# OpenRendererBenchmark/libYafaRay

Hardware: AMD Instinct MI355X
Metric: Mrays/sec (primary+secondary) on the path-tracing hot path (higher is better)
Workload: dtype f32; 1 GPU; 1M-tri diffuse Cornell-box soup 512x512 64spp primary+1-bounce (BASELINE.json metric config); triangles=1000000, width=512, height=512, spp=64, bounces=1, lights=1, parallelism=pixel-tile shard x1, film_reduce=none, kd_nodes=2803313, kd_leaf_refs=3155999, kd_max_depth=27

## Files before the change

libyafaray_amd/csrc/yafgpu_wavefront.h:

```cpp
#pragma once

namespace yafgpu {

constexpr int kWfRecs = 32;

struct WfArgs
{
	RenderArgs ra;
	float4 *state; uint32_t cap;
	float4 *results;
	uint32_t n_paths, pixel_begin, n_pixels;
	const uint32_t *pix_prefix;
	int frames;
	int frame_recs, has_glossy;
	int pix_listed;
	uint32_t *pix_xy;
	const uint32_t *q_closest_in, *q_shadow_in, *q_resume_in;
	uint32_t *q_closest_out, *q_shadow_out, *q_resume_out;
	uint32_t *verdict;
	float4 *shadow_filt;
	int replay, replay_lights;
	int ev_m;
	float4 *hit_cache; int hit_k;
	uint32_t *ev_flags;
// ... 1221 lines not shown
				if(!second && (gl & kGlSecond))
				{
					FREC(P, 9) = f4(gcol, f9.w);
					FREC(P, 6) = f4(v3(f6), fbits((gl & ~kGlSecond) | kGlOnSecond));
					wf_start_level(a, slot, c, v3(f2), v3(FREC(P, 3)));
					return W_PARK_CLOSEST;
				}
				if(second)
				{
					const float m_alpha = FREC(P, 1).x;
					alpha_p = rp.bg_transp_refract ? m_alpha + (1.f - m_alpha) * alpha : 1.f;
				}
			}
			else gcol = c3(f9) + (integ * c3(f10)) * f10.w;
			const int ns = (int)(gl & 0xffu) + 1, gsam = (int)((gl >> 8) & 0xffu);
			c.level = P;
			if(ns < gsam)
			{
				FREC(P, 9) = f4(gcol, f9.w);
				FREC(P, 6) = f4(v3(f6), fbits((uint32_t)ns | ((uint32_t)gsam << 8)));
				if(alpha_p != f0.w) FREC(P, 0) = f4(c3(f0), alpha_p);
				return W_GLOSSY_NEXT;
			}
			c.col = c3(f0) + gcol * (1.f / (float)gsam);
			VSET(3, f4(v3(f2), f9.w)); VSET(4, f4(v3(f6), 0.f)); VSET(5, FREC(P, 7)); VSET(6, FREC(P, 8));
			if(YAFGPU_FEAT_TEXTURE && a.ra.sc.tex.nodes != nullptr) REC(22) = FREC(P, 11);
			if(YAFGPU_FEAT_TEXTURE && a.ra.sc.tex.has_bump) REC(24) = FREC(P, 12);
			REC(19) = make_float4(0.f, 0.f, a.ev_m > 1 ? REC(19).z : 0.f, alpha_p);
			return W_RECURSE_SPEC;
		}
		if(flags & ((flags & 2u) ? 8u : 4u))
		{
			const yafgpu_material &pm = a.ra.sc.mats[ubits(FREC(P, 4).w)];
			integ = integ * beer_transmittance(pm.beer_sigma, FREC(P, 3).w);
		}
		if(!(flags & 2u))
		{
			const Col col_p = c3(f0) + integ * c3(FREC(P, 4));
			if(flags & 1u)
			{
				FREC(P, 0) = f4(col_p, f0.w);
				FREC(P, 2) = f4(v3(f2), fbits(2u | (flags & 8u) | (flags & 0xf00u)));
				wf_start_level(a, slot, c, wf_transp_origin(a.ra.sc.mats[ubits(FREC(P, 4).w)], v3(f2), v3(FREC(P, 3)), P + 1), v3(FREC(P, 3)));
				return W_PARK_CLOSEST;
			}
			c.col = col_p; alpha = f0.w;
		}
		else
		{
			const float4 f1 = FREC(P, 1);
			c.col = c3(f0) + integ * c3(f1);
			alpha = rp.bg_transp_refract ? f1.w + (1.f - f1.w) * alpha : 1.f;
		}
		c.level = P;
	}
}
#undef FREC

YG_DEV int wf_advance(const WfArgs &a, uint32_t slot, uint32_t pixel_sample, uint32_t sampling_offs, uint32_t ordinal, const float4 ans, float result[4], int &out_mask)
{
	Ctl c = load_ctl(a, slot);
	const bool beside = YAFGPU_FEAT_LIGHTS && c.pc == kPcAfterBoth;
	int where = (YAFGPU_FEAT_LIGHTS && (c.pc == kPcAfterShadow || beside)) ? W_AFTER_SHADOW : W_AFTER_CLOSEST;
	Hot h; hot_init(h);
	uint32_t w_last = 0u;
	float alpha = 0.f;
	uint2 verdict = make_uint2(0u, 0u), verdict2 = verdict;
	if(where == W_AFTER_SHADOW)
	{
		const uint32_t w = a.verdict[slot >> 3], sh = (slot & 7u) << 2;
		verdict = make_uint2((w >> sh) & 1u, (w >> (sh + 1u)) & 1u);
		verdict2 = make_uint2((w >> (sh + 2u)) & 1u, (w >> (sh + 3u)) & 1u);
		hot_preload(a, slot, h, c.stage != kStPrimary);
		if(YAFGPU_FEAT_LIGHTS && !beside)
		{
			const uint32_t w14 = ubits(h.r14.w);
			const int li = (int)(w14 & 0xffu), l_end = (int)((w14 >> 8) & 0xffu), is = (int)(w14 >> 20);
			bool more = li + 1 < l_end;
			if(YAFGPU_FEAT_AO && !more && li < l_end && li >= a.ra.sc.n_lights) more = is + 1 < ao_n_samples(a.ra.rp, wf_div(a, slot, c.level).division);
			else if(!more && li < l_end)
			{
				const yafgpu_light &light = a.ra.sc.lights[li];
				more = !light_is_dirac(light.type) && is + 1 < dl_area_samples(a.ra, light, wf_div(a, slot, c.level).division);
			}
			if(more) { if(c.dl_on_sp0) VNEED(3); else VNEED(7); }
		}
	}
	int pend2 = (YAFGPU_FEAT_LIGHTS && YAFGPU_FEAT_MULTI) ? c.mask2 : 0;
	c.mask2 = 0;
	if(beside)
	{
		where = st_after_shadow(a, slot, h, verdict);
		if(where == W_DL_NEXT) where = st_dl_next(a, slot, h, c.level);
		if(YAFGPU_FEAT_MULTI && where == W_DL_EVAL && pend2)
		{
			where = st_after_shadow(a, slot, h, verdict2, true, pend2);
			pend2 = 0;
			if(where == W_DL_NEXT) where = st_dl_next(a, slot, h, c.level);
		}
		if(where == W_DL_DONE) where = st_dl_done(a, slot, h, c, true);
		if(where == W_NEXT_VERTEX) where = W_AFTER_CLOSEST;
	}
	if(where == W_AFTER_CLOSEST) where = st_after_closest(a, slot, h, c, ordinal, ans, beside);
	if(YAFGPU_FEAT_LIGHTS && !a.vtx_lds && where == W_DL_NEXT) { if(c.dl_on_sp0) VNEED(3); else VNEED(7); }
	if(YAFGPU_FEAT_LIGHTS)
	{
		if(where == W_AFTER_SHADOW) where = st_after_shadow(a, slot, h, verdict);
		bool second = false;
		uint32_t w2 = 0u;
		while(where == W_DL_NEXT || where == W_DL_EVAL)
		{
			if(where == W_DL_NEXT) where = st_dl_next(a, slot, h, c.level);
			else if(YAFGPU_FEAT_MULTI && pend2) { where = st_after_shadow(a, slot, h, verdict2, true, pend2); pend2 = 0; }
			else
			{
				int m = 0;
				const int r = st_dl_eval(a, slot, h, c, pixel_sample, sampling_offs, m, second, w2);
				if(!second)
				{
					where = r;
					if(r == W_PARK_SHADOW)
					{
						out_mask = m;
						w_last = ubits(HGET(14).w);
						if(YAFGPU_FEAT_MULTI && a.multi)
						{
							const int li = (int)(w_last & 0xffu), l_end = (int)((w_last >> 8) & 0xffu), is = (int)(w_last >> 20);
							int n;
							if(YAFGPU_FEAT_AO && li >= a.ra.sc.n_lights) n = ao_n_samples(a.ra.rp, wf_div(a, slot, c.level).division);
							else
							{
								const yafgpu_light &light = a.ra.sc.lights[li];
								n = light_is_dirac(light.type) ? 1 : dl_area_samples(a.ra, light, wf_div(a, slot, c.level).division);
							}
							const bool same = is + 1 < n;
							if(same || li + 1 < l_end) { second = true; w2 = pack_dlc(same ? li : li + 1, l_end, 0, same ? is + 1 : 0); where = W_DL_EVAL; }
						}
					}
				}
				else
				{
					if(r == W_PARK_SHADOW) { c.mask2 = m; out_mask |= m << 2; w_last = w2; }
					where = W_PARK_SHADOW;
				}
			}
		}
	}
	if(where == W_DL_DONE) where = st_dl_done(a, slot, h, c, false);
	if(YAFGPU_FEAT_LIGHTS && where == W_PARK_SHADOW) where = st_beside(a, slot, h, c, pixel_sample, sampling_offs, ordinal, w_last);
	if(where == W_EXTEND) where = st_extend(a, slot, h, c);
	if(where == W_START_PATH) where = st_start_path(a, slot, h, c, pixel_sample, sampling_offs, ordinal);
	if(where == W_RECURSE) where = st_recurse(a, slot, h, c);
#if YAFGPU_FEAT_RECURSE
	for(;;)
	{
		if(where == W_GLOSSY_NEXT) where = st_glossy_next(a, slot, c, pixel_sample, sampling_offs);
		if(where == W_RECURSE_SPEC) where = st_recurse_spec(a, slot, h, c);
		if(where != W_RETURN) break;
		where = st_return(a, slot, h, c, alpha);
		if(where != W_GLOSSY_NEXT && where != W_RECURSE_SPEC) break;
	}
#else
	if(where == W_RETURN) where = st_return(a, slot, h, c, alpha);
#endif
	if(where != W_FINISH) hot_flush(a, slot, h, where == W_PARK_CLOSEST);
#if YAFGPU_FEAT_LIGHTS
	if(where != W_FINISH)
	{
		const bool sampler_later = c.stage == kStPrimary || (c.stage == kStFirst ? 1 : c.depth + 1) < a.ra.rp.bounces;
		vtx_flush(a, slot, h, where == W_PARK_SHADOW && sampler_later);
	}
#endif
	if(where == W_PARK_CLOSEST) { c.pc = kPcAfterClosest; REC(13) = f4(c.col, fbits(pack_ctl(c))); return kReqClosest; }
	if(where == W_PARK_SHADOW) { c.pc = kPcAfterShadow; REC(13) = f4(c.col, fbits(pack_ctl(c))); return kReqShadow; }
	if(where == W_PARK_BOTH) { c.pc = kPcAfterBoth; REC(13) = f4(c.col, fbits(pack_ctl(c))); return kReqBoth; }
	if(a.ra.rp.bg_transp) alpha = smax(alpha, 0.f);
	result[0] = c.col.r; result[1] = c.col.g; result[2] = c.col.b; result[3] = alpha;
	return kReqDone;
}
#ifdef YAFGPU_STEP_PROBE
#ifndef PROBE_WAVES
#define PROBE_WAVES 1
#endif
__global__ __launch_bounds__(kBlock, PROBE_WAVES) void probe_advance(const WfArgs a, int *out)
{
	const uint32_t slot = blockIdx.x * blockDim.x + threadIdx.x; float r[4] = {0.f, 0.f, 0.f, 0.f}; int m = 0;
	out[slot] = wf_advance(a, slot, slot * 3u, slot * 5u, slot * 7u, a.state[2 * (size_t)a.cap + slot], r, m) + m + (int)r[0] + (int)r[3];
}
#define PROBE(name, call) __global__ __launch_bounds__(kBlock, PROBE_WAVES) void name(const WfArgs a, int *out) { \
	const uint32_t slot = blockIdx.x * blockDim.x + threadIdx.x; Ctl c = load_ctl(a, slot); int m = 0; (void)m; \
	Hot h; hot_init(h); hot_preload(a, slot, h, true); const int w = call; hot_flush(a, slot, h, false); \
	a.state[(size_t)13 * a.cap + slot] = f4(c.col, fbits(pack_ctl(c))); out[slot] = w + m; }
PROBE(probe_after_closest, st_after_closest(a, slot, h, c, slot * 7u, a.state[2 * (size_t)a.cap + slot], false))
PROBE(probe_after_shadow, st_after_shadow(a, slot, h, make_uint2(slot & 1u, slot & 2u)))
PROBE(probe_dl_next, st_dl_next(a, slot, h, c.level))
PROBE(probe_dl_eval, st_dl_eval(a, slot, h, c, slot * 3u, slot * 5u, m))
PROBE(probe_dl_done, st_dl_done(a, slot, h, c, false))
PROBE(probe_extend, st_extend(a, slot, h, c))
PROBE(probe_start_path, st_start_path(a, slot, h, c, slot * 3u, slot * 5u, slot * 7u))
#undef PROBE
#endif

#undef REC

template<bool kTable>
YG_DEV void wf_identity(const WfArgs &a, uint32_t slot, int &px, int &py, int &sample, uint32_t &pixel_sample, uint32_t &sampling_offs, uint32_t &ordinal)
{
	const yafgpu_render_params &rp = a.ra.rp;
	const uint32_t spp = (uint32_t)rp.aa_minsamples;
	const uint32_t pixel_local = slot / spp;
	sample = (int)(slot - pixel_local * spp);
	if(kTable) { const uint32_t xy = a.pix_xy[pixel_local]; px = (int)(xy & 0xffffu); py = (int)(xy >> 16); }
	else wf_pixel_of(a, pixel_local, px, py);
	sampling_offs = fnv32a((uint32_t)py * fnv32a((uint32_t)px));
	pixel_sample = rp.base_sampling_offset + rp.pass_offset + (uint32_t)sample;
	ordinal = ((uint32_t)(py - rp.ystart) * (uint32_t)rp.width + (uint32_t)(px - rp.xstart)) * spp + (uint32_t)sample;
}

YG_DEV void wf_sample_offsets(const WfArgs &a, int sample, uint32_t sampling_offs, float &dx, float &dy)
{
	const int n_samples = a.ra.rp.aa_minsamples;
	dx = 0.5f; dy = 0.5f;
	if(a.ra.rp.multi_pass)
	{
		const uint32_t pixel_sample = a.ra.rp.base_sampling_offset + a.ra.rp.pass_offset + (uint32_t)sample;
		dx = ri_vdc(pixel_sample, sampling_offs);
		dy = ri_s(pixel_sample, sampling_offs);
	}
	else if(n_samples > 1)
	{
		const float d_1 = (float)(1.0 / (double)(float)n_samples);
		dx = (float)((0.5 + (double)(float)sample) * (double)d_1);
		dy = ri_lp((uint32_t)sample + sampling_offs, 0u);
	}
}

YG_DEV void wf_push(uint32_t *queue, uint32_t *count, bool pred, uint32_t slot)
{
	const unsigned long long mask = __ballot(pred);
	if(mask == 0ull) return;
	const int lane = (int)(threadIdx.x & (kWave - 1));
	const int leader = __ffsll((long long)mask) - 1;
	uint32_t base = 0u;
	if(lane == leader) base = atomicAdd(count, (uint32_t)__popcll(mask));
	base = (uint32_t)__shfl((int)base, leader, kWave);
	if(pred) queue[base + (uint32_t)__popcll(mask & ((1ull << lane) - 1ull))] = slot;
}

#ifndef YAFGPU_VARIANT_TU
template<bool kPanoramic>
__global__ __launch_bounds__(kBlock) void wf_generate(const WfArgs a)
{
	for(uint32_t slot = blockIdx.x * blockDim.x + threadIdx.x; slot < a.n_paths; slot += gridDim.x * blockDim.x)
	{
		int px, py, sample; uint32_t pixel_sample, sampling_offs, ordinal;
		if(a.pix_listed) wf_identity<true>(a, slot, px, py, sample, pixel_sample, sampling_offs, ordinal);
		else
		{
			wf_identity<false>(a, slot, px, py, sample, pixel_sample, sampling_offs, ordinal);
			if(sample == 0) a.pix_xy[slot / (uint32_t)a.ra.rp.aa_minsamples] = (uint32_t)px | ((uint32_t)py << 16);
		}
		float dx, dy;
		wf_sample_offsets(a, sample, sampling_offs, dx, dy);
		V3 from, dir; float tmin, tmax;
		float lens_u = 0.5f, lens_v = 0.5f;
		if(a.ra.sc.cam.aperture != 0.f)
		{
			Halton hal_u, hal_v;
			hal_u.init(3u); hal_v.init(5u);
			const uint32_t start = a.ra.rp.base_sampling_offset + a.ra.rp.pass_offset + sampling_offs;
			hal_u.set_start(start); hal_v.set_start(start);
			for(int k = 0; k <= sample; ++k) { lens_u = hal_u.next(); lens_v = hal_v.next(); }
		}
		float wt;
		camera_shoot<kPanoramic>(a.ra.sc.cam, (float)px + dx, (float)py + dy, lens_u, lens_v, from, dir, tmin, tmax, wt);
		const bool live = !kPanoramic || wt != 0.f;
		if(live)
		{
			float4 *b = a.state + slot; const size_t c = a.cap;
			b[0 * c] = f4(from, tmin);
			b[1 * c] = f4(dir, tmax);
			b[13 * c] = make_float4(0.f, 0.f, 0.f, fbits((uint32_t)kPcAfterClosest | ((uint32_t)kStPrimary << 2)));
		}
		else a.results[slot] = make_float4(0.f, 0.f, 0.f, 1.f);
		if(kPanoramic && a.q_closest_out != nullptr) wf_push(a.q_closest_out, &a.cnt_in[0], live, slot);
	}
	if((!kPanoramic || a.q_closest_out == nullptr) && blockIdx.x == 0 && threadIdx.x == 0) { a.cnt_in[0] = a.n_paths; a.cnt_in[1] = 0u; a.cnt_in[2] = 0u; a.cnt_in[3] = 0u; a.cnt_in[4] = 0u; }
}

#ifndef YAFGPU_VOTE_NUM
#define YAFGPU_VOTE_NUM 1
#endif
#ifndef YAFGPU_VOTE_DEN
#define YAFGPU_VOTE_DEN 1
#endif
#ifndef YAFGPU_NODE_BURST
#define YAFGPU_NODE_BURST 2
#endif
#ifndef YAFGPU_TRACE_BATCH
#define YAFGPU_TRACE_BATCH 512
#endif
constexpr int kTraceBatch = YAFGPU_TRACE_BATCH;
#ifndef YAFGPU_REFILL
#define YAFGPU_REFILL 24
#endif
#ifndef YAFGPU_TRACE_POSTPONE
#define YAFGPU_TRACE_POSTPONE 1
#endif
#ifndef YAFGPU_TRACE_BELOW_MASKS
#define YAFGPU_TRACE_BELOW_MASKS 1
#endif
#ifndef YAFGPU_TRACE_WAVES
#define YAFGPU_TRACE_WAVES 7
#endif
template<bool kAny, bool kStats>
__global__ __launch_bounds__(kBlock, YAFGPU_TRACE_WAVES) void wf_trace(const WfArgs a)
{
	__shared__ uint2 s_stack[kWavesPerBlock][kStack][kWave];
	__shared__ float2 s_axis[kWavesPerBlock][3][kWave];
	const int lane = (int)(threadIdx.x & (kWave - 1)), wave = (int)(threadIdx.x >> 6);
	const DevScene &sc = a.ra.sc;
	const uint32_t root = sc.tl_root;
	LaneStack stk;
	stk.col = &s_stack[wave][0][lane];
	float2 *const axis_col = &s_axis[wave][0][lane];
	LaneCounters cn = {0u, 0u, 0u, 0u, 0u, 0u, 0u};
	const uint32_t n = kAny ? a.cnt_in[1] : a.cnt_in[0];
	uint32_t *cursor = kAny ? &a.cnt_in[3] : &a.cnt_in[2];
	const uint32_t *q = kAny ? a.q_shadow_in : a.q_closest_in;
	const size_t c = a.cap;
	bool exhausted = (n == 0u);
	uint32_t slot = 0u, link = 0u, which = 0u, pair = 0u, qi = 0u;
	uint32_t w_next = 0u, w_end = 0u;
	const uint32_t batch = min((uint32_t)kTraceBatch, max((uint32_t)kWave, (n / (gridDim.x * (uint32_t)kWavesPerBlock * 2u)) & ~63u));
	V3 from = mk(0.f, 0.f, 0.f), dir = from;
	uint32_t dneg = 0u;
	float ray_tmin = 0.f, dist = 0.f, t_exit = 0.f, tmin = 0.f, tmax = 0.f, z = 0.f, bu = 0.f, bv = 0.f;
	int tri = -1; bool hit = false;
	auto answer_any = [&](bool occluded) {
		const uint32_t bit = 4u * slot + 2u * pair + which;
		if(occluded) atomicOr(&a.verdict[bit >> 5], 1u << (bit & 31u));
	};
	enum : uint32_t { kWalk = 0u, kBlocked = 1u, kWalkEnd = 2u, kNoRay = 3u };
	constexpr int kVoteNum = YAFGPU_VOTE_NUM, kVoteDen = YAFGPU_VOTE_DEN, kNodeBurst = YAFGPU_NODE_BURST;
	uint32_t ws = kNoRay;
	uint32_t p_cur = 0u, p_end = 0u, ti = 0u;
	float p_tmax = 0.f;
	bool done = false;
	uint32_t spec = 0u;
	uint32_t spec_leaves = 0u;
	uint32_t rounds_node = 0u, rounds_tri = 0u;
	for(;;)
	{
		const unsigned long long idle = __ballot(ws == kNoRay);
		const int n_idle = __popcll(idle);
		if(!exhausted && (n_idle >= YAFGPU_REFILL || n_idle == kWave))
		{
			if(w_next >= w_end)
			{
				const int leader = __ffsll((long long)idle) - 1;
				uint32_t base = 0u;
				if(lane == leader) base = atomicAdd(cursor, batch);
				base = (uint32_t)__shfl((int)base, leader, kWave);
				w_next = base; w_end = min(base + batch, n);
				if(base >= n) { exhausted = true; w_next = w_end = 0u; }
			}
			const uint32_t avail = w_end - w_next;
			const uint32_t rank = (uint32_t)__popcll(idle & ((1ull << lane) - 1ull));
			const uint32_t first_i = w_next;
			w_next += min(avail, (uint32_t)n_idle);
			if(ws == kNoRay && rank < avail)
			{
				const uint32_t i = first_i + rank;
				slot = q ? q[i] : i;
				qi = i;
				which = slot >> 31;
				pair = kAny ? (slot >> 30) & 1u : 0u;
				slot &= kAny ? 0x3fffffffu : 0x7fffffffu;
				float4 r0 = a.state[slot], r1 = a.state[c + slot];
				if(!kAny && which)
				{
					const float4 r26 = a.state[26 * c + slot];
					r1 = make_float4(r26.x, r26.y, r26.z, -1.f);
					r0.w = r26.w;
				}
				if(kAny && pair)
				{
					const float4 ra_ = a.state[(which ? 30 : 28) * c + slot];
					const float rb_ = a.state[(which ? 31 : 29) * c + slot].w;
					r1 = make_float4(ra_.x, ra_.y, ra_.z, which ? rb_ : ra_.w);
					r0.w = which ? ra_.w : rb_;
				}
				else if(kAny && which)
				{
					const float4 r20 = a.state[20 * c + slot];
					r1 = make_float4(r20.x, r20.y, r20.z, a.state[21 * c + slot].w);
					r0.w = r20.w;
				}
				from = v3(r0); dir = v3(r1);
				if(kAny)
				{
					from = from + dir * r0.w;
					dist = (r1.w < 0.f) ? INFINITY : r1.w - 2.f * r0.w;
					ray_tmin = a.ra.rp.transp_shad ? r0.w : 0.f;
					++cn.shadow;
				}
				else
				{
					dist = (r1.w < 0.f) ? INFINITY : r1.w;
					ray_tmin = r0.w;
					++cn.closest;
				}
				float ea, eb;
				tri = -1; hit = false; z = dist; bu = 0.f; bv = 0.f; done = false; p_cur = p_end = 0u;
				const V3 inv_dir = mk(1.f / dir.x, 1.f / dir.y, 1.f / dir.z);
				if(sc.n_nodes != 0u && bound_cross(sc, from, dir, inv_dir, dist, ea, eb) && !(dist < smax(ea, 0.f)))
				{
					axis_col[0] = make_float2(from.x, inv_dir.x);
					axis_col[kWave] = make_float2(from.y, inv_dir.y);
					axis_col[2 * kWave] = make_float2(from.z, inv_dir.z);
					dneg = (dir.x <= 0.f ? 1u : 0u) | (dir.y <= 0.f ? 2u : 0u) | (dir.z <= 0.f ? 4u : 0u);
					t_exit = eb; tmin = smax(ea, 0.f); tmax = t_exit; link = root; ws = kWalk;
					stk.reset();
				}
				else
				{
					if(!kAny) a.state[2 * c + qi] = make_float4(fbits(0xffffffffu), dist, 0.f, 0.f);
				}
			}
		}
		const unsigned long long m_act = __ballot(ws != kNoRay);
		if(m_act == 0ull) { if(exhausted) break; else continue; }
		const bool has_pend = p_cur < p_end;
		const unsigned long long m_tri = __ballot(has_pend);
		const int n_tri = __popcll(m_tri), n_node = __popcll(__ballot(ws == kWalk));
		auto leaf_end = [&]() {
			const uint2 top = stk.col[((stk.sp - 1) & (kStack - 1)) * kWave];
			const bool hit_here = !kAny && hit && z <= tmax;
			const bool emp = stk.empty();
			const bool restart = emp && stk.lost() && !(tmax >= t_exit);
			if(kStats && restart && !hit_here) ++cn.restarts;
			tmin = restart ? restart_from(tmin, tmax) : tmax;
			link = emp ? root : top.x;
			tmax = emp ? t_exit : __uint_as_float(top.y);
			stk.sp = emp ? 0 : stk.sp - 1;
			stk.lo = emp ? 0 : stk.lo;
			const bool fin = hit_here || (emp && !restart) || z < tmin;
			ws = fin ? kWalkEnd : kWalk;
		};
		auto tri_step = [&](const float4 r0, const float4 r1, const float4 r2, const uint32_t ref_v) {
			float t, u, v;
			if(kStats) ++cn.tests;
			const bool ok = tri_test_flat(r0, r1, r2, from, dir, t, u, v);
			const uint32_t vis = __float_as_uint(r1.w) >> 30;
			if(kAny)
			{
				const bool found = ok && t < dist && t >= ray_tmin && (vis == 0u || vis == 2u);
				hit = hit || found; done = done || found;
			}
			else
			{
				const bool better = ok && t < z && t >= ray_tmin && (vis == 0u || vis == 1u);
				z = better ? t : z; tri = better ? (int)ti : tri; bu = better ? u : bu; bv = better ? v : bv; hit = hit || better;
			}
			++p_cur; ti = ref_v;
			if(p_cur >= p_end)
			{
				if(YAFGPU_TRACE_POSTPONE)
				{
					const bool ends = !kAny && hit && z <= p_tmax;
					done = done || ends;
					if(kStats) { if(done) { cn.interior -= spec; cn.leaves -= spec_leaves; } spec = 0u; spec_leaves = 0u; }
					if(!kAny && ws != kWalkEnd && z < tmin) ws = kWalkEnd;
					ws = (ws == kBlocked) ? kWalk : ws;
				}
				else if(!done) leaf_end();
			}
		};
		auto node_step = [&](const uint4 t0, const uint4 t1) {
			const uint32_t sl = link & 3u;
			const uint32_t axis = (t0.w >> (2u * sl)) & 3u;
			const float split = __uint_as_float(sl == 0u ? t0.x : (sl == 1u ? t0.y : t0.z));
			const float2 oi = axis_col[axis * kWave];
			const float o = oi.x;
			const float tplane = (split - o) * oi.y;
			const bool dn = ((dneg >> axis) & 1u) != 0u;
#if YAFGPU_TRACE_BELOW_MASKS
			const bool below = __builtin_amdgcn_inverse_ballot_w64(__ballot(o < split) | (__ballot(o == split) & __ballot(dn)));
#else
			const bool below = dn ? (o <= split) : (o < split);
#endif
			const bool l_in = sl == 0u && ((t0.w >> 2) & 3u) != 3u, r_in = sl == 0u && ((t0.w >> 4) & 3u) != 3u;
			const uint32_t left = l_in ? (link | 1u) : (sl == 2u ? t1.z : t1.x);
			const uint32_t right = r_in ? (link | 2u) : (sl == 0u ? t1.z : (sl == 1u ? t1.y : t1.w));
			const uint32_t near_c = below ? left : right, far_c = below ? right : left;
			if(kStats) { ++cn.interior; if(p_cur < p_end) ++spec; }
			const bool near_only = !(tplane <= tmax) || tplane <= 0.f;
			const bool far_only = !near_only && tplane < tmin;
			const bool both = !near_only && !far_only;
			stk.col[(stk.sp & (kStack - 1)) * kWave] = make_uint2(far_c, __float_as_uint(tmax));
			stk.sp += both ? 1 : 0;
			stk.lo = max(stk.lo, stk.sp - (kStack - 1));
			link = far_only ? far_c : near_c;
			tmax = both ? tplane : tmax;
		};
		auto leaf_step = [&]() {
			uint32_t first = link & ((1u << kLinkFirstBits) - 1u), np = (link >> kLinkFirstBits) & kLinkCountMax;
			if(link & kLinkEscape) { const uint2 e = sc.tl_leaves[link & kLinkIndex]; first = e.x; np = e.y; }
			if(np == 0u) { if(kStats) { ++cn.leaves; if(p_cur < p_end) ++spec_leaves; } leaf_end(); }
			else if(!YAFGPU_TRACE_POSTPONE)
			{
				if(kStats) ++cn.leaves;
				p_cur = first; p_end = first + np; p_tmax = tmax; ti = sc.refs[first]; ws = kBlocked;
			}
			else if(p_cur < p_end) ws = kBlocked;
			else
			{
				if(kStats) ++cn.leaves;
				p_cur = first; p_end = first + np; p_tmax = tmax;
				ti = sc.refs[first];
				leaf_end();
			}
		};
		if(n_tri * kVoteNum >= n_node * kVoteDen && n_tri > 0)
		{
			if(kStats) ++rounds_tri;
			if(has_pend)
			{
				uint32_t ref_v = 0u;
				if(p_cur + 1u < p_end) ref_v = sc.refs[p_cur + 1u];
				const float4 r0 = sc.tri[3u * ti], r1 = sc.tri[3u * ti + 1u], r2 = sc.tri[3u * ti + 2u];
				tri_step(r0, r1, r2, ref_v);
			}
		}
		else
		{
#pragma unroll 1
			for(int s = 0; s < kNodeBurst; ++s)
			{
				if(kStats && __ballot(ws == kWalk) != 0ull) ++rounds_node;
				if(ws == kWalk && (link & kLinkLeaf)) leaf_step();
				const bool fetch = ws == kWalk && !(link & kLinkLeaf);
				const uint32_t at = link >> 2;
				uint4 t0 = make_uint4(0u, 0u, 0u, 0u), t1 = t0;
				if(fetch) { t0 = sc.treelets[2u * at]; t1 = sc.treelets[2u * at + 1u]; }
				if(fetch) node_step(t0, t1);
				if(ws == kWalk && (link & kLinkLeaf)) leaf_step();
				if(fetch && ws == kWalk && (link >> 2) == at) node_step(t0, t1);
			}
		}
		if(done || (ws == kWalkEnd && p_cur >= p_end))
		{
			if(kAny) answer_any(hit);
			else a.state[2 * c + qi] = make_float4(fbits((uint32_t)(hit ? tri : -1)), z, bu, bv);
			ws = kNoRay; done = false; p_cur = p_end = 0u;
		}
	}
	if(a.ra.counters != nullptr)
	{
		const uint32_t v0 = wave_sum(cn.closest), v1 = wave_sum(cn.shadow), v2 = wave_sum(cn.interior), v3_ = wave_sum(cn.leaves),
		               v4 = wave_sum(cn.tests), v6 = wave_sum(cn.restarts);
		if(lane == 0 && (v0 | v1))
		{
			if(v0) atomicAdd((unsigned long long *)&a.ra.counters->rays_closest, (unsigned long long)v0);
			if(v1) atomicAdd((unsigned long long *)&a.ra.counters->rays_shadow, (unsigned long long)v1);
			if(kStats)
			{
				atomicAdd((unsigned long long *)&a.ra.counters->interior_steps, (unsigned long long)v2);
				atomicAdd((unsigned long long *)&a.ra.counters->leaves, (unsigned long long)v3_);
				atomicAdd((unsigned long long *)&a.ra.counters->tri_tests, (unsigned long long)v4);
				atomicAdd((unsigned long long *)&a.ra.counters->restarts, (unsigned long long)v6);
				atomicAdd((unsigned long long *)&a.ra.counters->wave_rounds, (unsigned long long)rounds_node | ((unsigned long long)rounds_tri << 32));
			}
		}
	}
}


__global__ __launch_bounds__(kBlock) void wf_trace_ts(const WfArgs a)
{
	__shared__ uint2 s_stack[kWavesPerBlock][kStack][kWave];
	__shared__ uint32_t s_seen[kWavesPerBlock][kTsMaxDepth + 1][kWave];
	const int lane = (int)(threadIdx.x & (kWave - 1)), wave = (int)(threadIdx.x >> 6);
	const DevScene &sc = a.ra.sc;
	LaneStack stk;
	stk.col = &s_stack[wave][0][lane];
	uint32_t *seen = &s_seen[wave][0][lane];
	const uint32_t n = a.cnt_in[1];
	const size_t c = a.cap;
	uint32_t count = 0u;
	for(uint32_t i = blockIdx.x * blockDim.x + threadIdx.x; i < n; i += gridDim.x * blockDim.x)
	{
		uint32_t slot = a.q_shadow_in[i];
		const uint32_t which = slot >> 31; slot &= 0x7fffffffu;
		float4 r0 = a.state[slot], r1 = a.state[c + slot];
		if(which)
		{
			const float4 r20 = a.state[20 * c + slot];
			r1 = make_float4(r20.x, r20.y, r20.z, a.state[21 * c + slot].w);
			r0.w = r20.w;
		}
		const V3 dir = v3(r1);
		const V3 from = v3(r0) + dir * r0.w;
		const float dist = (r1.w < 0.f) ? INFINITY : r1.w - 2.f * r0.w;
		Col filt;
		const bool sh = kd_trace_ts(sc, stk, seen, from, dir, r0.w, dist, a.ra.rp.shadow_depth, filt);
		if(sh) { const uint32_t bit = 4u * slot + which; atomicOr(&a.verdict[bit >> 5], 1u << (bit & 31u)); }
		a.shadow_filt[2u * slot + which] = f4(filt, 0.f);
		++count;
	}
	if(a.ra.counters != nullptr)
	{
		const uint32_t v = wave_sum(count);
		if(lane == 0 && v) atomicAdd((unsigned long long *)&a.ra.counters->rays_shadow, (unsigned long long)v);
	}
}

#endif
#ifndef YAFGPU_SHADE_WAVES
#define YAFGPU_SHADE_WAVES 3
#endif
#ifndef YAFGPU_SHADE_LDS_TABLES
#define YAFGPU_SHADE_LDS_TABLES 1
#endif
constexpr int kShadeTabBytes = 16384;
#ifndef YAFGPU_SHADE_LDS_FAURE
#define YAFGPU_SHADE_LDS_FAURE 1
#endif
constexpr int kShadeFaureBytes = YAFGPU_SHADE_LDS_FAURE ? 8192 : 0;
__global__ __launch_bounds__(kBlock, YAFGPU_SHADE_WAVES) void wf_shade(const WfArgs a_in)
{
#if YAFGPU_SHADE_LDS_TABLES
	__shared__ uint4 s_tab[(kShadeTabBytes + kShadeFaureBytes) / 16];
	WfArgs a = a_in;
	if(YAFGPU_SHADE_LDS_FAURE)
	{
		int *dst = (int *)s_tab + kShadeTabBytes / 4;
		const uint32_t n_near = min((uint32_t)a_in.ra.sc.n_faure, (uint32_t)kShadeFaureBytes / 4u);
		for(uint32_t w = threadIdx.x; w < n_near; w += blockDim.x) dst[w] = a_in.ra.sc.faure[w];
		a.ra.sc.faure = dst; a.ra.sc.faure_near = (int)n_near;
		__syncthreads();
	}
	{
		const uint32_t mat_bytes = (uint32_t)a_in.ra.sc.n_mats * (uint32_t)sizeof(yafgpu_material);
		const uint32_t light_off = (mat_bytes + 15u) & ~15u;
		const uint32_t light_bytes = (uint32_t)a_in.ra.sc.n_lights * (uint32_t)sizeof(yafgpu_light);
		if(light_off + light_bytes <= (uint32_t)kShadeTabBytes)
		{
			uint32_t *dst = (uint32_t *)s_tab;
			const uint32_t *src_m = (const uint32_t *)a_in.ra.sc.mats, *src_l = (const uint32_t *)a_in.ra.sc.lights;
			for(uint32_t w = threadIdx.x; w < mat_bytes / 4u; w += blockDim.x) dst[w] = src_m[w];
			for(uint32_t w = threadIdx.x; w < light_bytes / 4u; w += blockDim.x) dst[light_off / 4u + w] = src_l[w];
			__syncthreads();
			a.ra.sc.mats = (const yafgpu_material *)s_tab;
			a.ra.sc.lights = (const yafgpu_light *)((const char *)s_tab + light_off);
		}
	}
#else
	const WfArgs &a = a_in;
#endif
	constexpr int kItems = 4;
	__shared__ uint32_t s_tot[kWavesPerBlock][3];
	__shared__ uint32_t s_base[kWavesPerBlock][3];
	__shared__ uint32_t s_item[kItems][kBlock];
	__shared__ uint8_t s_more[kItems][kBlock];
	const int lane = (int)(threadIdx.x & (kWave - 1)), wave = (int)(threadIdx.x >> 6);
	const uint32_t nc = a.cnt_in[0], nr = a.cnt_in[4];
	const uint32_t total = nc + nr;
	if(YAFGPU_FEAT_LIGHTS && a.replay == 2 && a.hit_cache != nullptr && a.ra.counters != nullptr && blockIdx.x == 0 && threadIdx.x == 0 && nc)
		atomicAdd((unsigned long long *)&a.ra.counters->rays_closest, (unsigned long long)nc);
	const uint32_t per_block = (uint32_t)kBlock * kItems;
	for(uint32_t base = blockIdx.x * per_block; base < total; base += gridDim.x * per_block)
	{
		uint32_t wc = 0u, wr = 0u, ws = 0u;
#pragma unroll 1
		for(int k = 0; k < kItems; ++k)
		{
			const uint32_t i = base + (uint32_t)k * kBlock + threadIdx.x;
			const bool live = i < total;
			int code = 0, more = 0;
			uint32_t slot = 0u;
			if(live)
			{
				slot = (i < nc) ? (a.q_closest_in ? (a.q_closest_in[i] & 0x7fffffffu) : i) : a.q_resume_in[i - nc];
				float4 ans = make_float4(0.f, 0.f, 0.f, 0.f);
				if(i < nc)
				{
					if(YAFGPU_FEAT_LIGHTS && a.replay == 2 && a.hit_cache != nullptr)
					{
						uint32_t ctl = ubits(wf_rec(a, 13, slot).w);
						if(a.q_closest_in && (a.q_closest_in[i] >> 31)) ctl = wf_ctl_of_beside(ctl);
						const uint32_t z19 = a.ev_m > 1 ? ubits(wf_rec(a, 19, slot).z) : 0u;
						ans = a.hit_cache[wf_hit_key(a, slot, ctl, z19)];
					}
					else ans = a.state[2 * (size_t)a.cap + i];
				}
				int px, py, sample; uint32_t pixel_sample, sampling_offs, ordinal;
				wf_identity<true>(a, slot, px, py, sample, pixel_sample, sampling_offs, ordinal);
				float res[4];
				int m = 0;
				const int req = wf_advance(a, slot, pixel_sample, sampling_offs, ordinal, ans, res, m);
				if(req == kReqDone)
				{
					if(res[3] > 1.f) res[3] = 1.f;
					a.results[slot] = make_float4(res[0], res[1], res[2], res[3]);
				}
				else if(req == kReqClosest) code = 1;
				else if(req == kReqShadow) code = 2 | ((m & 1) ? 4 : 0) | ((m & 2) ? 8 : 0);
				else if(req == kReqBoth) code = 1 | 16 | ((m & 1) ? 4 : 0) | ((m & 2) ? 8 : 0);
				if(req == kReqShadow || req == kReqBoth) more = (m >> 2) & 3;
			}
			s_item[k][threadIdx.x] = slot | ((uint32_t)code << 27);
			s_more[k][threadIdx.x] = (uint8_t)more;
			wc += (uint32_t)__popcll(__ballot(code & 1));
			wr += (uint32_t)__popcll(__ballot(code & 2));
			ws += (uint32_t)__popcll(__ballot(code & 4)) + (uint32_t)__popcll(__ballot(code & 8)) + (uint32_t)__popcll(__ballot(more & 1)) + (uint32_t)__popcll(__ballot(more & 2));
		}
		if(lane == 0) { s_tot[wave][0] = wc; s_tot[wave][1] = wr; s_tot[wave][2] = ws; }
		__syncthreads();
		if(threadIdx.x < 3)
		{
			const int qi = (int)threadIdx.x;
			uint32_t sum = 0u;
			for(int w = 0; w < kWavesPerBlock; ++w) sum += s_tot[w][qi];
			uint32_t b = 0u;
			if(sum) b = atomicAdd(&a.cnt_out[qi == 0 ? 0 : (qi == 1 ? 4 : 1)], sum);
			for(int w = 0; w < kWavesPerBlock; ++w) { s_base[w][qi] = b; b += s_tot[w][qi]; }
		}
		__syncthreads();
		uint32_t oc = s_base[wave][0], orr = s_base[wave][1], os = s_base[wave][2];
		const unsigned long long below = (1ull << lane) - 1ull;
#pragma unroll
		for(int k = 0; k < kItems; ++k)
		{
			const uint32_t item = s_item[k][threadIdx.x];
			const int code = (int)(item >> 27);
			const uint32_t slot = item & 0x07ffffffu;
			const unsigned long long bc = __ballot(code & 1), br = __ballot(code & 2), ba = __ballot(code & 4), bb = __ballot(code & 8);
			if(code & 1) a.q_closest_out[oc + (uint32_t)__popcll(bc & below)] = slot | ((code & 16) ? 0x80000000u : 0u);
			if(code & 2) a.q_resume_out[orr + (uint32_t)__popcll(br & below)] = slot;
			if(code & 4) a.q_shadow_out[os + (uint32_t)__popcll(ba & below)] = slot;
			const uint32_t na = (uint32_t)__popcll(ba);
			if(code & 8) a.q_shadow_out[os + na + (uint32_t)__popcll(bb & below)] = slot | 0x80000000u;
			os += na + (uint32_t)__popcll(bb);
			const int more = (int)s_more[k][threadIdx.x];
			const unsigned long long b2a = __ballot(more & 1), b2b = __ballot(more & 2);
			if(b2a | b2b)
			{
				if(more & 1) a.q_shadow_out[os + (uint32_t)__popcll(b2a & below)] = slot | 0x40000000u;
				const uint32_t n2a = (uint32_t)__popcll(b2a);
				if(more & 2) a.q_shadow_out[os + n2a + (uint32_t)__popcll(b2b & below)] = slot | 0xc0000000u;
				os += n2a + (uint32_t)__popcll(b2b);
			}
			oc += (uint32_t)__popcll(bc); orr += (uint32_t)__popcll(br);
		}
		__syncthreads();
	}
}

YG_DEV float4 wf_clamped(float4 c, float max_value)
{
	if(max_value > 0.f)
	{
		const float max_rgb = smax(c.x, smax(c.y, c.z));
		const float adj = max_value / max_rgb;
		if(max_rgb > max_value)
		{
			if(c.x >= max_rgb) { c.x = max_value; c.y *= adj; c.z *= adj; }
			else if(c.y >= max_rgb) { c.y = max_value; c.x *= adj; c.z *= adj; }
			else { c.z = max_value; c.x *= adj; c.y *= adj; }
		}
	}
	return c;
}

#ifndef YAFGPU_VARIANT_TU
__global__ __launch_bounds__(kBlock) void wf_accumulate(const WfArgs a)
{
	const yafgpu_render_params &rp = a.ra.rp;
	const int spp = rp.aa_minsamples;
	const int cx1 = rp.xstart + rp.width, cy1 = rp.ystart + rp.height;
	const size_t plane_stride = (size_t)rp.width * (size_t)rp.height * YAFGPU_FILM_CHANNELS;
	for(uint32_t pl = blockIdx.x * blockDim.x + threadIdx.x; pl < a.n_pixels; pl += gridDim.x * blockDim.x)
	{
		const uint32_t xy = a.pix_xy[pl];
		const int px = (int)(xy & 0xffffu), py = (int)(xy >> 16);
		const uint32_t sampling_offs = fnv32a((uint32_t)py * fnv32a((uint32_t)px));
		if(a.ra.wide_filter)
		{
			const int cx0 = rp.xstart, cy0 = rp.ystart;
			const double fw = (double)a.ra.filterw, ts = (double)a.ra.table_scale;
			float own[YAFGPU_FILM_CHANNELS] = {0.f, 0.f, 0.f, 0.f, 0.f};
			for(int s = 0; s < spp; ++s)
			{
				const float4 r = wf_clamped(a.results[(size_t)pl * (size_t)spp + (size_t)s], rp.aa_clamp_samples);
				float dx, dy;
				wf_sample_offsets(a, s, sampling_offs, dx, dy);
				const int dx_0 = max(cx0 - px, round2int((double)dx - fw)), dx_1 = min(cx1 - px - 1, round2int((double)dx + fw - 1.0));
				const int dy_0 = max(cy0 - py, round2int((double)dy - fw)), dy_1 = min(cy1 - py - 1, round2int((double)dy + fw - 1.0));
				const double x_offs = (double)dx - 0.5, y_offs = (double)dy - 0.5;
				for(int j = dy_0; j <= dy_1; ++j)
				{
					const int yi = (int)floor(fabs(((double)j - y_offs) * ts));
					for(int i = dx_0; i <= dx_1; ++i)
					{
						const int xi = (int)floor(fabs(((double)i - x_offs) * ts));
						const float w = a.ra.filter_table[yi * 16 + xi];
						if(i == 0 && j == 0)
						{
							own[0] += r.x * w; own[1] += r.y * w; own[2] += r.z * w; own[3] += r.w * w; own[4] += w;
						}
						else
						{
							float *dst = a.ra.planes + ((size_t)(py + j - cy0) * (size_t)rp.width + (size_t)(px + i - cx0)) * YAFGPU_FILM_CHANNELS;
							atomicAdd(dst + 0, r.x * w); atomicAdd(dst + 1, r.y * w); atomicAdd(dst + 2, r.z * w); atomicAdd(dst + 3, r.w * w);
							atomicAdd(dst + 4, w);
						}
					}
				}
			}
			float *dst = a.ra.planes + ((size_t)(py - cy0) * (size_t)rp.width + (size_t)(px - cx0)) * YAFGPU_FILM_CHANNELS;
#pragma unroll
			for(int c = 0; c < YAFGPU_FILM_CHANNELS; ++c) atomicAdd(dst + c, own[c]);
			continue;
		}
		const size_t pix = ((size_t)(py - rp.ystart) * (size_t)rp.width + (size_t)(px - rp.xstart)) * YAFGPU_FILM_CHANNELS;
		float acc[YAFGPU_FILM_PLANES][YAFGPU_FILM_CHANNELS];
#pragma unroll
		for(int k = 0; k < YAFGPU_FILM_PLANES; ++k)
#pragma unroll
			for(int c = 0; c < YAFGPU_FILM_CHANNELS; ++c) acc[k][c] = rp.accumulate ? a.ra.planes[(size_t)k * plane_stride + pix + c] : 0.f;
		for(int s = 0; s < spp; ++s)
		{
			const float4 r = wf_clamped(a.results[(size_t)pl * (size_t)spp + (size_t)s], rp.aa_clamp_samples);
			float dx, dy;
			wf_sample_offsets(a, s, sampling_offs, dx, dy);
			const int dx_1 = min(cx1 - px - 1, round2int((double)dx + (double)a.ra.filterw - 1.0));
			const int dy_1 = min(cy1 - py - 1, round2int((double)dy + (double)a.ra.filterw - 1.0));
			acc[0][0] += r.x; acc[0][1] += r.y; acc[0][2] += r.z; acc[0][3] += r.w; acc[0][4] += 1.f;
			if(dx_1 >= 1) { acc[1][0] += r.x; acc[1][1] += r.y; acc[1][2] += r.z; acc[1][3] += r.w; acc[1][4] += 1.f; }
			if(dy_1 >= 1) { acc[2][0] += r.x; acc[2][1] += r.y; acc[2][2] += r.z; acc[2][3] += r.w; acc[2][4] += 1.f; }
			if(dx_1 >= 1 && dy_1 >= 1) { acc[3][0] += r.x; acc[3][1] += r.y; acc[3][2] += r.z; acc[3][3] += r.w; acc[3][4] += 1.f; }
		}
#pragma unroll
		for(int k = 0; k < YAFGPU_FILM_PLANES; ++k)
		{
			if(k == 0 || acc[k][4] != 0.f)
			{
				float *dst = a.ra.planes + (size_t)k * plane_stride + pix;
#pragma unroll
				for(int c = 0; c < YAFGPU_FILM_CHANNELS; ++c) dst[c] = acc[k][c];
			}
		}
	}
	if(a.ra.counters != nullptr && blockIdx.x == 0 && threadIdx.x == 0)
		atomicAdd((unsigned long long *)&a.ra.counters->camera_samples, (unsigned long long)a.n_paths);
}

// ... 132 lines not shown
```

Before: 2635 Mrays/s.

## Defer trace result writes until refill and pin visibility word

Adds a kAnswer state so a finished ray's result store (closest-hit state write, or atomicOr for an occluded shadow ray) is held until the next wave-wide refill step and then issued together, instead of scattered at each lane's completion. The refill threshold rises from 24 to 32 idle lanes. An inline asm barrier pins the visibility word extraction to steer instruction scheduling in the triangle test. An optional stats mode that counts occluded shadow rays is also added. The aim is fewer divergent memory ops inside the traversal loop, at the cost of holding results longer and refilling less often.

```diff
diff --git a/libyafaray_amd/csrc/yafgpu_wavefront.h b/libyafaray_amd/csrc/yafgpu_wavefront.h
--- a/libyafaray_amd/csrc/yafgpu_wavefront.h
+++ b/libyafaray_amd/csrc/yafgpu_wavefront.h
@@ -1547,13 +1547,25 @@
 #endif
 constexpr int kTraceBatch = YAFGPU_TRACE_BATCH;
 #ifndef YAFGPU_REFILL
-#define YAFGPU_REFILL 24
+#define YAFGPU_REFILL 32
 #endif
 #ifndef YAFGPU_TRACE_POSTPONE
 #define YAFGPU_TRACE_POSTPONE 1
 #endif
 #ifndef YAFGPU_TRACE_BELOW_MASKS
 #define YAFGPU_TRACE_BELOW_MASKS 1
+#endif
+#ifndef YAFGPU_TRACE_DEFER_ANY
+#define YAFGPU_TRACE_DEFER_ANY 1
+#endif
+#ifndef YAFGPU_TRACE_DEFER_CLOSEST
+#define YAFGPU_TRACE_DEFER_CLOSEST 1
+#endif
+#ifndef YAFGPU_TRACE_VIS_PIN
+#define YAFGPU_TRACE_VIS_PIN 1
+#endif
+#ifndef YAFGPU_STATS_OCCLUDED
+#define YAFGPU_STATS_OCCLUDED 0
 #endif
 #ifndef YAFGPU_TRACE_WAVES
 #define YAFGPU_TRACE_WAVES 7
@@ -1586,7 +1598,12 @@
 		const uint32_t bit = 4u * slot + 2u * pair + which;
 		if(occluded) atomicOr(&a.verdict[bit >> 5], 1u << (bit & 31u));
 	};
-	enum : uint32_t { kWalk = 0u, kBlocked = 1u, kWalkEnd = 2u, kNoRay = 3u };
+	enum : uint32_t { kWalk = 0u, kBlocked = 1u, kWalkEnd = 2u, kNoRay = 3u, kAnswer = 4u };
+	constexpr bool kDefer = kAny ? (YAFGPU_TRACE_DEFER_ANY != 0) : (YAFGPU_TRACE_DEFER_CLOSEST != 0);
+	auto answer = [&]() {
+		if(kAny) answer_any(hit);
+		else a.state[2 * c + qi] = make_float4(fbits((uint32_t)(hit ? tri : -1)), z, bu, bv);
+	};
 	constexpr int kVoteNum = YAFGPU_VOTE_NUM, kVoteDen = YAFGPU_VOTE_DEN, kNodeBurst = YAFGPU_NODE_BURST;
 	uint32_t ws = kNoRay;
 	uint32_t p_cur = 0u, p_end = 0u, ti = 0u;
@@ -1597,10 +1614,11 @@
 	uint32_t rounds_node = 0u, rounds_tri = 0u;
 	for(;;)
 	{
-		const unsigned long long idle = __ballot(ws == kNoRay);
+		const unsigned long long idle = __ballot(ws >= kNoRay);
 		const int n_idle = __popcll(idle);
 		if(!exhausted && (n_idle >= YAFGPU_REFILL || n_idle == kWave))
 		{
+			if(kDefer && ws == kAnswer) { answer(); ws = kNoRay; }
 			if(w_next >= w_end)
 			{
 				const int leader = __ffsll((long long)idle) - 1;
@@ -1674,7 +1692,7 @@
 				}
 			}
 		}
-		const unsigned long long m_act = __ballot(ws != kNoRay);
+		const unsigned long long m_act = __ballot(ws < kNoRay);
 		if(m_act == 0ull) { if(exhausted) break; else continue; }
 		const bool has_pend = p_cur < p_end;
 		const unsigned long long m_tri = __ballot(has_pend);
@@ -1684,7 +1702,7 @@
 			const bool hit_here = !kAny && hit && z <= tmax;
 			const bool emp = stk.empty();
 			const bool restart = emp && stk.lost() && !(tmax >= t_exit);
-			if(kStats && restart && !hit_here) ++cn.restarts;
+			if(kStats && !YAFGPU_STATS_OCCLUDED && restart && !hit_here) ++cn.restarts;
 			tmin = restart ? restart_from(tmin, tmax) : tmax;
 			link = emp ? root : top.x;
 			tmax = emp ? t_exit : __uint_as_float(top.y);
@@ -1697,7 +1715,13 @@
 			float t, u, v;
 			if(kStats) ++cn.tests;
 			const bool ok = tri_test_flat(r0, r1, r2, from, dir, t, u, v);
+#if YAFGPU_TRACE_VIS_PIN
+			uint32_t vis_w = __float_as_uint(r1.w);
+			asm volatile("; visibility word of the record" : "+v"(vis_w));
+			const uint32_t vis = vis_w >> 30;
+#else
 			const uint32_t vis = __float_as_uint(r1.w) >> 30;
+#endif
 			if(kAny)
 			{
 				const bool found = ok && t < dist && t >= ray_tmin && (vis == 0u || vis == 2u);
@@ -1796,9 +1820,10 @@
 		}
 		if(done || (ws == kWalkEnd && p_cur >= p_end))
 		{
-			if(kAny) answer_any(hit);
-			else a.state[2 * c + qi] = make_float4(fbits((uint32_t)(hit ? tri : -1)), z, bu, bv);
-			ws = kNoRay; done = false; p_cur = p_end = 0u;
+			if(kStats && YAFGPU_STATS_OCCLUDED && kAny && hit) ++cn.restarts;
+			const bool hold = kDefer && !exhausted && (!kAny || hit);
+			if(!hold) answer();
+			ws = hold ? kAnswer : kNoRay; done = false; p_cur = p_end = 0u;
 		}
 	}
 	if(a.ra.counters != nullptr)
```

Result: faster. 2697 Mrays/s, median of 6 (+2.4%).
